# ictnlp/StreamSpeech

Hardware: AMD Instinct MI355X
Metric: real-time factor (RTFx = audio seconds / wall seconds) + utterances/sec, offline S2ST fr-en (higher is better)
Workload: dtype f32

## Files before the change

### include/streamspeech_hip.h

```cpp
#ifndef STREAMSPEECH_HIP_H
#define STREAMSPEECH_HIP_H

#include <stddef.h>
#include <stdint.h>

#ifdef __cplusplus
extern "C" {
#endif

#define SS_ABI_VERSION 2

typedef struct ss_model ss_model;
typedef struct ss_vocoder ss_vocoder;
typedef struct ss_scratch ss_scratch;
typedef struct ss_stream_pool ss_stream_pool;

typedef struct ss_config {
  int32_t input_feat, conv_channels, conv_kernel;
  int32_t enc_dim, enc_ffn, enc_heads, enc_layers, dw_kernel;
  int32_t src_vocab, tgt_vocab;
  int32_t mt_layers, dec_dim, dec_ffn, dec_heads;
  int32_t t2u_layers, unit_layers, unit_vocab, ctc_upsample;
  int32_t pad, eos, unk;
  int32_t max_rel_pos;
// ... 379 lines not shown
                          int64_t* h_attn_off, int64_t attn_capacity, int32_t* d_peak, float* d_stat);
int ss_batch_vocoder_tail(ss_vocoder* v, void* stream, int B, const int32_t* d_codes, const int32_t* h_K, const int32_t* h_n_new,
                          const int32_t* h_ctx, const int32_t* h_rf, int dur_prediction, float* d_out, int64_t out_capacity,
                          int32_t* h_win_first, int32_t* h_dur, int64_t* h_out_start, int64_t* h_n_out);
int ss_batch_vocoder_tail_spkr(ss_vocoder* v, void* stream, int B, const int32_t* d_codes, const int32_t* h_K, const int32_t* h_n_new,
                               const int32_t* h_ctx, const int32_t* h_rf, int dur_prediction, float* d_out, int64_t out_capacity,
                               int32_t* h_win_first, int32_t* h_dur, int64_t* h_out_start, int64_t* h_n_out,
                               const int32_t* h_spkr );

int ss_prof_enable(int cls_mask);
int ss_prof_enable_hi(int cls_mask);
int ss_prof_reset(void);
int ss_prof_read(int cls, double* h_ms_total, double* h_flops_total, int64_t* h_launches,
                 double* h_bytes_total);
int ss_prof_totals(int cls, double* h_flops_total, double* h_bytes_total, int64_t* h_launches);
int ss_prof_read_issued(int cls, double* h_issued_flops_total);
int ss_prof_shape_log(int on);
int ss_prof_shape_dump(char* buf, int cap);
int ss_prof_num_classes(void);
const char* ss_prof_class_name(int cls);

int ss_model_set_pack_invariant(ss_model* m, int on);
int ss_model_get_pack_invariant(ss_model* m);
int ss_debug_canon(int mode);

int ss_debug_last_logits(ss_model* m, void* stream, float* d_out, int64_t cap_floats, int* h_rows, int* h_cols);

int ss_op_ffn_fused(void* stream, const float* dX, int ldx, float* dY, int ldy, const float* ln_g, const float* ln_b,
                    const float* dW1, const float* db1, const float* dW2, const float* db2, float alpha,
                    const float* ln2_g, const float* ln2_b, int M, int D, int F);
int ss_debug_ffn(int grid, int row_tiles_per_wave, int enable);
int ss_debug_rtlin(int grid, int enable);
int ss_debug_conv_c64(int enable);
int ss_debug_conv_c32(int enable);
int ss_debug_conv_c16(int enable);
int64_t ss_debug_enc_step_launches(void);
int ss_op_ln_linear(void* stream, const float* dX, int ldx, const float* ln_g, const float* ln_b, const float* dW,
                    const float* dbias, const float* dR, int ldr, float* dC, int ldc, int M, int N, int K, int act, float alpha,
                    int glu);

int ss_debug_force_tile(int bm, int bn, int ks);
int ss_debug_sk_errors(void);
int ss_debug_attention_split(int v);
int ss_debug_attention_q16(int v);
int ss_debug_enc_step_inject_timeout(ss_model* m);
int ss_debug_scratch_audit(ss_scratch* sc, size_t* booked, size_t* held);
int ss_debug_mt_inject_timeout(ss_model* m);

int ss_op_conv_gemm(void* stream, const float* dA, int lda, const float* dW, const float* dbias,
                    const float* dR, int ldr, const float* dR2, int ldr2, float* dC, int ldc,
                    int M, int N, int Cin, int taps, int dil, int stride, int pad, int in_len,
                    int chunk, int in_act, float in_slope, int act, float alpha, float div, int glu);
typedef struct ss_op_conv_args {
  const float* A; const float* W; const float* bias; const float* R; const float* R2; float* C; float* C2;
  int32_t lda, ldc, ldr, ldr2, ldc2;
  int32_t M, N, Cin, taps, dil, stride, pad, in_len, chunk;
  int32_t in_act; float in_slope;
  int32_t act; float act_slope, alpha, div, c2_slope;
  int32_t glu;
  const int32_t* segs; int32_t nseg, max_seg_out;
  int32_t same_rows;
} ss_op_conv_args;
int ss_op_conv_gemm_ex(void* stream, const ss_op_conv_args* a);
int ss_op_conv_gemm_rows(void* stream, const ss_op_conv_args* a, int m_begin, const int32_t* seg_mb, const float* const* seg_A, int canon);
int ss_op_conv_pair(void* stream, const float* dA, int lda, const float* dW1, const float* db1, const float* dW2, const float* db2,
                    float* dC, int ldc, const float* dR2, int ldr2, float div, float* dC2, int ldc2, float c2_slope, int C, int taps,
// ... 121 lines not shown
```

### streamspeech_amd/csrc/conv_c64w.hip

```cpp
#include "slab_common.hpp"

#include <type_traits>

namespace ss {

using u32x4 = __attribute__((ext_vector_type(4))) unsigned;

#ifndef CW_TIMING
#define CW_TIMING 0
#endif
#if CW_TIMING
__device__ unsigned long long g_cw_dbg[1024 * 8];
#define CW_STAMP(k) do { if (t == 0) { const unsigned long long _n = __builtin_amdgcn_s_memtime(); cw_acc[k] += _n - cw_last; cw_last = _n; } } while (0)
#else
#define CW_STAMP(k) do { } while (0)
#endif

namespace {
constexpr int CW_MAXSEG = 256;
constexpr int CW_MAXROWS = 320;
[[maybe_unused]] constexpr int CW_NUM_RECORDS = 0x7ffffff0;
constexpr int cw_bme(int dil) { return dil == 1 ? 256 : dil == 3 ? 252 : 240; }
[[maybe_unused]] __host__ __device__ constexpr int cw_nc(int kind) { return kind == 0 ? 4 : kind == 1 ? 2 : 3; }
[[maybe_unused]] __host__ __device__ constexpr int cw_slot(int kind, int n) { return kind == 0 ? n : kind == 1 ? (n == 0 ? 0 : 3) : (n == 2 ? 3 : n); }
[[maybe_unused]] __host__ __device__ constexpr int cw_ja(int kind, int n) { return kind == 0 ? (n == 3 ? 1 : n) : kind == 1 ? n : (n == 0 ? 0 : 1); }
[[maybe_unused]] __host__ __device__ constexpr int cw_jb(int kind, int n) { return kind == 0 ? (n == 2 ? 1 : n == 3 ? 3 : 2) : kind == 1 ? n : (n == 2 ? 2 : 1); }
[[maybe_unused]] __host__ __device__ constexpr int cw_op(int kind, int n) { return kind == 0 ? (n == 1 ? 1 : -1) : kind == 1 ? 0 : (n == 1 ? 0 : -1); }
}

__global__ void wino_pack_kernel(const float* __restrict__ W, float* __restrict__ WW, int C, int taps, int groups) {
  const int n = C * groups * C;
  for (int idx = blockIdx.x * blockDim.x + threadIdx.x; idx < n; idx += gridDim.x * blockDim.x) {
    const int ci = idx % C, g = (idx / C) % groups, co = idx / (C * groups);
    const float* w = W + (size_t)co * taps * C + ci;
    const float w0 = 3 * g < taps ? w[(size_t)(3 * g) * C] : 0.f;
    const float w1 = 3 * g + 1 < taps ? w[(size_t)(3 * g + 1) * C] : 0.f;
    const float w2 = 3 * g + 2 < taps ? w[(size_t)(3 * g + 2) * C] : 0.f;
    float* o = WW + (size_t)co * groups * 4 * C + (size_t)g * 4 * C + ci;
    const int left = taps - 3 * g;
    if (left >= 3) {
      o[0] = w0;
      o[C] = 0.5f * ((w0 + w1) + w2);
      o[2 * C] = 0.5f * ((w0 - w1) + w2);
      o[3 * C] = w2;
    } else if (left == 2) {
      o[0] = w0; o[C] = w0 + w1; o[2 * C] = 0.f; o[3 * C] = w1;
    } else {
      o[0] = w0; o[C] = 0.f; o[2 * C] = 0.f; o[3 * C] = -w0;
    }
  }
}

template <int DIL, int CH, int TAIL>
__global__ __launch_bounds__(CH >= 128 ? 512 : 256, CH >= 128 ? 1 : CH == 64 ? 2 : 3) void conv_c64w_kernel(const GemmArgs p, const int groups, const int slab_rows) {
#if __HIP_DEVICE_COMPILE__
  constexpr int CS = CH == 256 ? 128 : CH;
  constexpr int KH = CH / CS;
  constexpr int C = CH, LDA = CS + 4, CT = CH >= 64 ? 4 : CH / 16, CB = CS / 16, RING = 2 * CT, TPR = CS / 4;
  constexpr int NT = CH >= 128 ? 512 : 256, RPP = NT / TPR;
  constexpr int NP = (CW_MAXROWS + RPP - 1) / RPP, NPC = CH == 256 ? 10 : NP < 20 ? NP : 20, BME = cw_bme(DIL), NPAIR = BME / 2;
  extern __shared__ __attribute__((aligned(16))) float smem[];
  float* sA = smem;
  int* s_blk = reinterpret_cast<int*>(smem + ((slab_rows * LDA + 3) & ~3));

  const int t = threadIdx.x, lane = t & 63;
  const int wave = __builtin_amdgcn_readfirstlane((t >> 6) & 3);
  const int cs = CH <= 64 ? 0 : __builtin_amdgcn_readfirstlane(t >> 8);
  const int colh = CH == 256 ? (int)((blockIdx.x >> 3) & 1) : 0;
  const int col0 = colh * 128 + cs * 64;
  const int r = lane & 15, g = lane >> 4;
  const int Kw = groups * 4 * C;

  SlabWalk<GemmArgs> w(p, s_blk, BME);
  __syncthreads();
  const int nblocks = w.nblocks();
  const float slope = p.in_act == ACT_LRELU ? p.in_slope : 1.0f;

  const __amdgpu_buffer_rsrc_t rsW = __builtin_amdgcn_make_buffer_rsrc((void*)p.W, 0, CW_NUM_RECORDS, 0x00020000);
  const int vo = (r * Kw + 4 * g) * 4;
  auto wload = [&](int idx, int cc, int ct, int kh) -> f32x4 {
    const int so = __builtin_amdgcn_readfirstlane(((col0 + ct * 16) * Kw + idx * C + kh * CS + cc * 16) * 4);
    const u32x4 v = __builtin_amdgcn_raw_buffer_load_b128(rsW, vo, so, 0);
    return f32x4{__uint_as_float(v[0]), __uint_as_float(v[1]), __uint_as_float(v[2]), __uint_as_float(v[3])};
  };

  int blk = CH == 256 ? (int)((blockIdx.x & 7) + 8 * (blockIdx.x >> 4)) : (int)blockIdx.x;
  const int blk_stride = CH == 256 ? (int)(gridDim.x >> 1) : (int)gridDim.x;
  if (blk >= nblocks) return;
  f32x4 ring[RING];
#pragma unroll
  for (int q = 0; q < RING; ++q) ring[q] = wload(q / CT, 0, q % CT, 0);

  int toff[2];
  bool pv[2];
#pragma unroll
  for (int i = 0; i < 2; ++i) {
    const int pp = wave * 32 + i * 16 + r;
    pv[i] = pp < NPAIR;
    const int pc = pv[i] ? pp : NPAIR - 1;
    toff[i] = 2 * DIL * (pc / DIL) + pc % DIL;
  }

#if CW_TIMING
  unsigned long long cw_acc[4] = {0, 0, 0, 0}, cw_last = __builtin_amdgcn_s_memtime(), cw_begin = cw_last, cw_blocks = 0;
#endif
  for (; blk < nblocks; blk += blk_stride) {
#if CW_TIMING
    ++cw_blocks;
#endif
    w.locate(blk, p.in_len);
    const int m0 = w.m0, seg_lo = w.seg_lo, seg_hi = w.seg_hi;
    const int m_hi = p.nseg > 0 ? seg_hi : min(seg_hi, p.M);
    const bool edge = (m0 - p.pad < seg_lo) || (m0 - p.pad + slab_rows > seg_hi);
    f32x4 acc[4][2][CT];
#pragma unroll
    for (int f = 0; f < 4; ++f)
#pragma unroll
      for (int i = 0; i < 2; ++i)
#pragma unroll
        for (int j = 0; j < CT; ++j) acc[f][i][j] = f32x4{0.f, 0.f, 0.f, 0.f};
#pragma unroll 1
    for (int kh = 0; kh < KH; ++kh) {
    const int kh_wrap = kh + 1 < KH ? kh + 1 : 0;
    __syncthreads();
    CW_STAMP(kh == 0 ? 3 : 1);
#pragma unroll 1
    for (int u0 = 0; u0 < NP; u0 += NPC) {
      f32x4 pre[NPC];
#pragma unroll
      for (int u = 0; u < NPC; ++u) {
        const int rho = t / TPR + RPP * (u0 + u);
        const int gc = min(max(m0 - p.pad + rho, seg_lo), seg_hi - 1);
        pre[u] = *reinterpret_cast<const f32x4*>(p.A + (size_t)gc * p.lda + kh * CS + (t % TPR) * 4);
      }
      float* dst = sA + (t / TPR + RPP * u0) * LDA + (t % TPR) * 4;
#pragma unroll
      for (int u = 0; u < NPC; ++u) {
        const int rho = t / TPR + RPP * (u0 + u);
        f32x4 v = pre[u];
        if (edge) {
          const int gin = m0 - p.pad + rho;
          const bool ok = gin >= seg_lo && gin < seg_hi;
#pragma unroll
          for (int e = 0; e < 4; ++e) v[e] = ok ? v[e] : 0.f;
        }
#pragma unroll
        for (int e = 0; e < 4; ++e) v[e] = fmaxf(v[e], v[e] * slope);
        if (rho < slab_rows) *reinterpret_cast<f32x4*>(dst + u * RPP * LDA) = v;
      }
    }
    __syncthreads();
    CW_STAMP(0);

    const float* pa0 = sA + toff[0] * LDA + 4 * g;
    const float* pa1 = sA + toff[1] * LDA + 4 * g;
    auto rd = [&](const float* base, int j, int cc) -> f32x4 { return *reinterpret_cast<const f32x4*>(base + j * DIL * LDA + cc * 16); };
    auto xform = [&](int op, const f32x4 a, const f32x4 b) -> f32x4 { return op == 1 ? a + b : op == 0 ? a : a - b; };
    f32x4 xa[2];
    xa[0] = xform(-1, rd(pa0, 0, 0), rd(pa0, 2, 0));
    xa[1] = xform(-1, rd(pa1, 0, 0), rd(pa1, 2, 0));
    auto group = [&](auto KIND, const int grp, const int kind_next, const float* pn0, const float* pn1, const int grp_next, const int kh_next) __attribute__((always_inline)) {
      constexpr int K = decltype(KIND)::value, NC = cw_nc(K), NS = CB * NC;
      static_assert(NS % 2 == 0 && NS >= 2, "ring slots keep their parity across groups");
#pragma unroll
      for (int ss = 0; ss < NS; ++ss) {
// ... 85 lines not shown
        for (int j = 0; j < CT; ++j) slab_epi_store<CH >= 128>(p, mrow[q], cole + j * 16, y[q * CT + j]);
      }
    }
    CW_STAMP(2);
  }
#if CW_TIMING
  if (t == 0) {
    unsigned long long* d = g_cw_dbg + (size_t)(blockIdx.x & 1023) * 8;
    d[0] = cw_acc[0]; d[1] = cw_acc[1]; d[2] = cw_acc[2]; d[3] = cw_acc[3]; d[4] = cw_blocks; d[5] = cw_begin; d[6] = __builtin_amdgcn_s_memtime(); d[7] = 1;
  }
#endif
#endif
}

#if CW_TIMING
extern "C" int ss_debug_cw_timing(unsigned long long* h_out, int cap_wgs) {
  const int n = cap_wgs < 1024 ? cap_wgs : 1024;
  if (hipMemcpyFromSymbol(h_out, HIP_SYMBOL(g_cw_dbg), (size_t)n * 8 * sizeof(unsigned long long)) != hipSuccess) return -1;
  static unsigned long long zeros[1024 * 8];
  (void)hipMemcpyToSymbol(HIP_SYMBOL(g_cw_dbg), zeros, sizeof(zeros));
  return n;
}
#endif

void conv_c64w_debug(int enable) { if (enable >= 0) dispatch_edit([enable](Dispatch& d) { d.c64w_on = enable ? 1 : 0; }); }
bool conv_c64w_enabled() { return disp().c64w_on != 0; }
void conv_c128w_debug(int enable) { if (enable >= 0) dispatch_edit([enable](Dispatch& d) { d.c128w_on = enable ? 1 : 0; }); }
bool conv_c128w_enabled() { return disp().c128w_on != 0; }

void conv_c256w_debug(int enable) { if (enable >= 0) dispatch_edit([enable](Dispatch& d) { d.c256w_on = enable ? 1 : 0; }); }
bool conv_c256w_enabled() { return disp().c256w_on != 0; }

static int cw_groups(const GemmArgs& a) { return (a.taps + 2) / 3; }
static size_t cw_lds(const GemmArgs& a, int ch) { return slab_lds_bytes(cw_bme(a.dil) + 3 * cw_groups(a) * a.dil, ch + 4, CW_MAXSEG); }

bool conv_c64w_eligible(const GemmArgs& a) {
  if (!disp().c64w_on || !a.Wwino || a.taps < disp().c64w_min_k || a.taps < 3 || (a.dil != 1 && a.dil != 3 && a.dil != 5) || a.C2) return false;
  if (a.pad != a.dil * (a.taps - 1) / 2) return false;
  if (a.taps <= 8 && a.taps > 3 && a.dil == 5) return false;
  const int slab_rows = cw_bme(a.dil) + 3 * cw_groups(a) * a.dil;
  return slab_rows <= CW_MAXROWS && 2 * cw_lds(a, 64) <= 158 * 1024 && (size_t)cw_groups(a) * 4 * 64 * 64 * 4 < 0x7ff00000ull;
}

bool conv_wide_winograd_eligible(const GemmArgs& a, int ch) {
  if (ch != 128 && ch != 256) return false;
  const Dispatch& d = disp();
  if (!(ch == 128 ? d.c128w_on : d.c256w_on) || !a.Wwino || !slab_conv_ok(a, ch)) return false;
  if (a.taps < 3 || (a.dil != 1 && a.dil != 3 && a.dil != 5) || a.pad != a.dil * (a.taps - 1) / 2) return false;
  if (a.nseg > CW_MAXSEG || a.M < (ch == 128 ? d.c128w_min_rows : d.c256w_min_rows) || !slab_rows_ok(a.M)) return false;
  if (ch == 256 && (size_t)256 * cw_groups(a) * 4 * 256 * 4 >= 0x7ff00000ull) return false;
  const int slab_rows = cw_bme(a.dil) + 3 * cw_groups(a) * a.dil;
  return slab_rows <= CW_MAXROWS && cw_lds(a, 128) <= 160 * 1024;
}

int launch_wino_pack(const float* W, float* WW, int C, int taps, hipStream_t stream) {
  const int groups = (taps + 2) / 3, n = C * groups * C;
  hipLaunchKernelGGL(wino_pack_kernel, dim3((n + 255) / 256), dim3(256), 0, stream, W, WW, C, taps, groups);
  SS_LAUNCH_CHECK();
  return SS_OK;
}

template <int DIL, int CH, int TAIL>
static int launch_cw_t(GemmArgs a, hipStream_t stream) {
  constexpr int BME = cw_bme(DIL);
  const int groups = cw_groups(a);
  const int slab_rows = BME + 3 * groups * DIL;
  const size_t lds = cw_lds(a, CH == 256 ? 128 : CH);
  SS_MAX_LDS_ONCE((&conv_c64w_kernel<DIL, CH, TAIL>), CH >= 128 ? 160 * 1024 : 96 * 1024);
  SkWorkspace* st = nullptr;
  int rc = sk_workspace_acquire(stream, &st);
  if (rc != SS_OK) return rc;
  int grid = slab_grid(CH >= 128 ? 1 : CH == 64 ? 2 : 3, st->cus, a.M, BME, a.nseg);
  if (CH == 256) {
    long long want = std::min<long long>(st->cus, 2 * ((slab_max_blocks(a.M, BME, a.nseg) + 7) / 8 * 8));
    if (disp().slab_grid_cap > 0) want = std::min<long long>(want, disp().slab_grid_cap);
    grid = (int)std::max<long long>(16, want / 16 * 16);
  }
  ProfRec rec{}; bool prof = false;
  rc = prof_begin(a, stream, CH == 64 ? PROF_CONV_C64W : CH == 128 ? PROF_CONV_C128W : CH == 256 ? PROF_CONV_C256W : PROF_CONV_C32W, rec, prof);
  if (rc != SS_OK) return rc;
  a.W = a.Wwino;
  hipLaunchKernelGGL((conv_c64w_kernel<DIL, CH, TAIL>), dim3(grid), dim3(CH >= 128 ? 512 : 256), lds, stream, a, groups, slab_rows);
  SS_LAUNCH_CHECK();
  return prof_end(stream, rec, prof);
}

template <int CH>
static int launch_cw(const GemmArgs& a, hipStream_t stream) {
  if (a.in_act != ACT_NONE && a.in_act != ACT_LRELU) return SS_ERR_ARG;
  const int key = a.dil * 10 + a.taps % 3;
  switch (key) {
    case 10: return launch_cw_t<1, CH, 0>(a, stream);
    case 11: return launch_cw_t<1, CH, 1>(a, stream);
    case 12: return launch_cw_t<1, CH, 2>(a, stream);
    case 30: return launch_cw_t<3, CH, 0>(a, stream);
    case 31: return launch_cw_t<3, CH, 1>(a, stream);
    case 32: return launch_cw_t<3, CH, 2>(a, stream);
    case 50: return launch_cw_t<5, CH, 0>(a, stream);
    case 51: return launch_cw_t<5, CH, 1>(a, stream);
    case 52: return launch_cw_t<5, CH, 2>(a, stream);
    default: return SS_ERR_ARG;
  }
}

int launch_conv_c64w(const GemmArgs& a, hipStream_t stream) {
  if (!conv_c64_eligible(a) || !conv_c64w_eligible(a)) return SS_ERR_ARG;
  return launch_cw<64>(a, stream);
}
void conv_c32w_debug(int enable) { if (enable >= 0) dispatch_edit([enable](Dispatch& d) { d.c32w_on = enable ? 1 : 0; }); }
bool conv_c32w_enabled() { return disp().c32w_on != 0; }
bool conv_c32w_eligible(const GemmArgs& a) {
  if (!disp().c32w_on || !a.Wwino || a.taps < 3 || (a.dil != 1 && a.dil != 3 && a.dil != 5) || a.C2) return false;
  if (a.pad != a.dil * (a.taps - 1) / 2) return false;
  const int slab_rows = cw_bme(a.dil) + 3 * cw_groups(a) * a.dil;
  return slab_rows <= CW_MAXROWS && 3 * cw_lds(a, 32) <= 158 * 1024;
// ... 16 lines not shown
```

### streamspeech_amd/csrc/debug_ops.hip

```cpp
#include "model_internal.hpp"

static int op_bind_wino(GemmArgs& a, void* stream) {
  static thread_local std::map<hipStream_t, DevBuf> wino_tmps;
  DevBuf& wino_tmp = wino_tmps[(hipStream_t)stream];
  const int N = a.N, Cin = a.Cin, taps = a.taps;
  if ((conv_c64w_enabled() && N == 64 && Cin == 64 && taps >= 3 && conv_c64_eligible(a)) ||
      (conv_c128w_enabled() && N == 128 && Cin == 128 && taps >= 3 && a.same_rows && !a.glu) ||
      (conv_c256w_enabled() && N == 256 && Cin == 256 && taps >= 3 && a.same_rows && !a.glu) ||
      (conv_c32w_enabled() && N == 32 && Cin == 32 && taps >= 3 && conv_c32_eligible(a))) {
    RET(wino_tmp.ensure((size_t)N * ((taps + 2) / 3) * 4 * N * sizeof(float)));
    RET(launch_wino_pack(a.W, wino_tmp.f(), N, taps, (hipStream_t)stream));
    a.Wwino = wino_tmp.f();
  }
  return SS_OK;
}

extern "C" int ss_op_conv_gemm(void* stream, const float* dA, int lda, const float* dW, const float* dbias,
                               const float* dR, int ldr, const float* dR2, int ldr2, float* dC, int ldc, int M,
                               int N, int Cin, int taps, int dil, int stride, int pad, int in_len, int chunk,
                               int in_act, float in_slope, int act, float alpha, float div, int glu) {
  GemmArgs a;
  a.A = dA; a.lda = lda; a.W = dW; a.bias = dbias; a.R = dR; a.ldr = ldr; a.R2 = dR2; a.ldr2 = ldr2; a.C = dC; a.ldc = ldc;
  a.M = M; a.N = N; a.Cin = Cin; a.taps = taps; a.dil = dil; a.stride = stride; a.pad = pad; a.in_len = in_len;
  a.chunk = chunk; a.in_act = in_act; a.in_slope = in_slope; a.act = act; a.alpha = alpha; a.div = div; a.glu = glu;
// ... 73 lines not shown
  if (!m->sc->dbg_logits || cap_floats < (int64_t)m->sc->dbg_rows * m->sc->dbg_cols) return SS_ERR_CAPACITY;
  SS_HIP_CHECK(hipMemcpyAsync(d_out, m->sc->dbg_logits, (size_t)m->sc->dbg_rows * m->sc->dbg_cols * sizeof(float), hipMemcpyDeviceToDevice,
                              (hipStream_t)stream));
  return SS_OK;
}

extern "C" int ss_op_ffn_fused(void* stream, const float* dX, int ldx, float* dY, int ldy, const float* ln_g, const float* ln_b,
                               const float* dW1, const float* db1, const float* dW2, const float* db2, float alpha,
                               const float* ln2_g, const float* ln2_b, int M, int D, int F) {
  return launch_ffn_fused(dX, ldx, dY, ldy, ln_g, ln_b, dW1, db1, dW2, db2, alpha, ln2_g, ln2_b, M, D, F, (hipStream_t)stream,
                          canon_mode() == CANON_SEQ);
}
extern "C" int ss_debug_canon(int mode) {
  if (mode < 0 || mode > 2) return SS_ERR_ARG;
  canon_debug_set(mode);
  return SS_OK;
}
extern "C" int ss_op_ln_linear(void* stream, const float* dX, int ldx, const float* ln_g, const float* ln_b, const float* dW,
                               const float* dbias, const float* dR, int ldr, float* dC, int ldc, int M, int N, int K, int act,
                               float alpha, int glu) {
  GemmArgs a;
  a.A = dX; a.lda = ldx; a.W = dW; a.bias = dbias; a.R = dR; a.ldr = ldr; a.C = dC; a.ldc = ldc;
  a.M = M; a.N = N; a.Cin = K; a.in_len = M; a.act = act; a.alpha = alpha; a.glu = glu; a.same_rows = 1;
  a.ln_g = ln_g; a.ln_b = ln_b;
  return launch_conv_gemm(a, (hipStream_t)stream);
}
extern "C" int ss_debug_conv_c64(int enable) {
  if (enable == 4 || enable == 5) { conv_c64w_debug(enable == 5); return SS_OK; }
  if (enable == 6 || enable == 7) { conv_c128w_debug(enable == 7); return SS_OK; }
  if (enable == 8 || enable == 9) { conv_c256w_debug(enable == 9); return SS_OK; }
  conv_c64_debug(enable);
  return SS_OK;
}
extern "C" int ss_debug_conv_c32(int enable) {
  if (enable == 4 || enable == 5) { conv_c32w_debug(enable == 5); return SS_OK; }
  conv_c32_debug(enable);
  return SS_OK;
}
extern "C" int ss_debug_conv_c16(int enable) { conv_c16_debug(enable); return SS_OK; }
extern "C" int64_t ss_debug_enc_step_launches(void) { return (int64_t)enc_step_launch_count(); }
extern "C" int ss_debug_scratch_audit(ss_scratch* sc, size_t* booked, size_t* held) {
  if (!sc || !booked || !held) return SS_ERR_ARG;
  size_t sum = 0;
  bool foreign = false;
  for (DevBuf* b : sc->all()) {
    sum += b->bytes;
    if (b->acct != &sc->acct) foreign = true;
  }
  *booked = sc->acct.used;
  *held = sum;
  return foreign ? SS_ERR_ARG : SS_OK;
}
extern "C" int ss_debug_rtlin(int grid, int enable) {
  if (grid < 0) return SS_ERR_ARG;
  rtlin_debug(grid, enable);
  return SS_OK;
}
extern "C" int ss_debug_ffn(int grid, int row_tiles_per_wave, int enable) {
  if (grid < 0 || row_tiles_per_wave < -1 || row_tiles_per_wave > 4) return SS_ERR_ARG;
  ffn_fused_debug_grid(grid);
  ffn_fused_debug_rows(row_tiles_per_wave);
  if (enable >= 0) dispatch_edit([enable](Dispatch& d) { d.ffn_fusion = enable ? 1 : 0; });
  return SS_OK;
}

extern "C" int ss_op_layernorm(void* stream, const float* dx, int ldx, float* dy, int ldy, const float* dg,
// ... 169 lines not shown
```

### streamspeech_amd/csrc/dispatch.hpp

```cpp
#pragma once
#include <functional>

namespace ss {

struct Dispatch {
  int attn_no_mfma = 0;
  int attn_q16 = 1;
  int attn_split = 0;
  int c16_off = 0, c32_off = 0, c64_off = 0;
  long long c16_min_rows = 131072, c32_min_rows = 65536, c64_min_rows = 32768;
  int c64w_on = 1, c128w_on = 1, c256w_on = 1, c32w_on = 1;
  int c64w_min_k = 3;
  long long c128w_min_rows = 65536, c256w_min_rows = 32768;
  int slab_grid_cap = 0;
  int sk_groups = 0;
  int ffn_force_g = 0;
  int ffn_wm = 3, ffn_wm_forced = 0;
  int ffn_fusion = 1;
  int ffn_min_rows = 1000;
  int force_bm = 0, force_bn = 0, force_ks = 0;
  double sk_min_flops = 4e9;
  int no_resblock_fusion = 0, no_pair_fusion = 0;
  int rt_off = 0, rt_min_rows = 193, rt_force_g = 0;
  long long rt_min_units = 4000;
  long long rt_kb_min_units = 256;
  int rt_kb_xmap = 1;
  int rt_kb_uw = 0;
};

const Dispatch& disp();
void dispatch_edit(const std::function<void(Dispatch&)>& fn);

struct CtxDispatch {
  Dispatch d;
  unsigned gen = 0xffffffffu;
  const Dispatch* refresh();
};
struct DispatchScope {
  explicit DispatchScope(const Dispatch* d);
  ~DispatchScope();
  const Dispatch* prev;
};

}
```

### streamspeech_amd/csrc/gemm.hip

```cpp
#include "gemm.hpp"

#include <atomic>
#include <cstdio>
#include <cstdlib>
#include <cstring>
#include <map>
#include <string>
#include <mutex>
#include <tuple>
#include <type_traits>
#include <utility>
#include <vector>

namespace ss {

using f32x4 = __attribute__((ext_vector_type(4))) float;

template <int BM, int BN, int BK, int WM, int WN, int KS, int PD, bool BLK = false>
__global__ __launch_bounds__(256 * KS) void conv_gemm_kernel(const GemmArgs p) {
  static_assert(WM * WN == 4, "4 waves per k-group");
  static_assert(!BLK || KS == 1, "the blocked chain is the KS = 1 form");
  constexpr int LDK = BK + 8;
  constexpr int WTM = BM / WM, WTN = BN / WN;
  constexpr int TM = WTM / 16, TN = WTN / 16;
// ... 761 lines not shown
  SkWorkspace* w = new SkWorkspace();
  std::lock_guard<std::mutex> lk(g_skw_mu);
  g_skw_live.push_back(w);
  return w;
}
void sk_workspace_free(SkWorkspace* w) {
  if (!w) return;
  {
    std::lock_guard<std::mutex> lk(g_skw_mu);
    for (size_t i = 0; i < g_skw_live.size(); ++i)
      if (g_skw_live[i] == w) { g_skw_live.erase(g_skw_live.begin() + i); break; }
  }
  if (w->ws) (void)hipFree(w->ws);
  if (w->sync1) (void)hipFree(w->sync1);
  if (w->sync2) (void)hipFree(w->sync2);
  if (w->sync3) (void)hipFree(w->sync3);
  if (w->dbg) (void)hipFree(w->dbg);
  delete w;
}
namespace {
std::mutex g_disp_mu;
std::atomic<unsigned> g_disp_gen{1};
Dispatch env_defaults() {
  Dispatch d;
  auto I = [](const char* k, int dflt) { const char* e = getenv(k); return e ? atoi(e) : dflt; };
  auto L = [](const char* k, long long dflt) { const char* e = getenv(k); return e ? atoll(e) : dflt; };
  d.attn_split = I("SS_ATTN_NO_SPLIT", 0) ? -1 : 0; d.attn_q16 = I("SS_ATTN_Q16", d.attn_q16);
  d.c16_off = I("SS_NO_CONV_C16", 0) ? 1 : 0; d.c32_off = I("SS_NO_CONV_C32", 0) ? 1 : 0; d.c64_off = I("SS_NO_CONV_C64", 0) ? 1 : 0;
  d.c16_min_rows = L("SS_CONV_C16_MIN_ROWS", d.c16_min_rows); d.c32_min_rows = L("SS_CONV_C32_MIN_ROWS", d.c32_min_rows);
  d.c64_min_rows = L("SS_CONV_C64_MIN_ROWS", d.c64_min_rows);
  d.c64w_on = I("SS_CONV_C64_WINOGRAD", 1); d.c128w_on = I("SS_CONV_C128_WINOGRAD", 1); d.c256w_on = I("SS_CONV_C256_WINOGRAD", 1);
  d.c32w_on = I("SS_CONV_C32_WINOGRAD", 1); d.c64w_min_k = I("SS_CONV_C64_WINOGRAD_MIN_K", 3);
  d.c128w_min_rows = L("SS_CONV_C128_MIN_ROWS", d.c128w_min_rows); d.c256w_min_rows = L("SS_CONV_C256_MIN_ROWS", d.c256w_min_rows);
  if (getenv("SS_FFN_WM")) { d.ffn_wm = I("SS_FFN_WM", 3); d.ffn_wm_forced = 1; }
  d.ffn_fusion = I("SS_NO_FFN_FUSION", 0) ? 0 : 1; d.ffn_min_rows = I("SS_FFN_MIN_ROWS", d.ffn_min_rows);
  if (getenv("SS_SK_MIN_GFLOP")) d.sk_min_flops = 1e9 * atof(getenv("SS_SK_MIN_GFLOP"));
  d.no_resblock_fusion = I("SS_NO_RESBLOCK_FUSION", 0); d.no_pair_fusion = I("SS_NO_PAIR_FUSION", 0);
  d.rt_off = I("SS_NO_RTLIN", 0) ? 1 : 0; d.rt_min_rows = I("SS_RTLIN_MIN_ROWS", d.rt_min_rows); d.rt_min_units = L("SS_RTLIN_MIN_UNITS", d.rt_min_units);
  d.rt_kb_min_units = L("SS_RTLIN_KB_MIN_UNITS", d.rt_kb_min_units); d.rt_kb_uw = I("SS_RTLIN_KB_UW", d.rt_kb_uw); d.rt_kb_xmap = I("SS_RTLIN_KB_XMAP", d.rt_kb_xmap);
  return d;
}
Dispatch& process_settings() { static Dispatch d = env_defaults(); return d; }
thread_local const Dispatch* t_disp = nullptr;
thread_local CtxDispatch t_disp_own;
}
void dispatch_edit(const std::function<void(Dispatch&)>& fn) {
  std::lock_guard<std::mutex> lk(g_disp_mu);
  fn(process_settings());
  g_disp_gen.fetch_add(1, std::memory_order_release);
}
void slab_debug(int grid, long long min_rows) {
  const Dispatch dflt = env_defaults();
  dispatch_edit([=](Dispatch& d) {
    d.slab_grid_cap = grid > 0 ? grid : 0;
    const bool set = min_rows >= 0;
    d.c16_min_rows = set ? min_rows : dflt.c16_min_rows; d.c32_min_rows = set ? min_rows : dflt.c32_min_rows;
    d.c64_min_rows = set ? min_rows : dflt.c64_min_rows;
    d.c128w_min_rows = set ? min_rows : dflt.c128w_min_rows; d.c256w_min_rows = set ? min_rows : dflt.c256w_min_rows;
  });
}
const Dispatch* CtxDispatch::refresh() {
  const unsigned now = g_disp_gen.load(std::memory_order_acquire);
  if (gen != now) {
    std::lock_guard<std::mutex> lk(g_disp_mu);
    d = process_settings();
    gen = g_disp_gen.load(std::memory_order_relaxed);
  }
  return &d;
}
const Dispatch& disp() { return t_disp ? *t_disp : *t_disp_own.refresh(); }
DispatchScope::DispatchScope(const Dispatch* d) : prev(t_disp) { t_disp = d; }
DispatchScope::~DispatchScope() { t_disp = prev; }

SkScope::SkScope(SkWorkspace* w) : prev(t_skw), prev_disp(t_disp) { t_skw = w; t_disp = w ? w->disp.refresh() : nullptr; }
SkScope::~SkScope() { t_skw = prev; t_disp = prev_disp; }

int sk_workspace_acquire(hipStream_t stream, SkWorkspace** out) {
  *out = nullptr;
  int dev = 0;
  SS_HIP_CHECK(hipGetDevice(&dev));
  SkWorkspace* w = t_skw;
  if (!w) {
    std::lock_guard<std::mutex> lk(g_skw_mu);
    SkWorkspace*& slot = g_skw_fallback[std::make_pair(dev, stream)];
    if (!slot) { slot = new SkWorkspace(); g_skw_live.push_back(slot); }
    w = slot;
  }
  if (!w->ws) {
    int cus = 0;
    SS_HIP_CHECK(hipDeviceGetAttribute(&cus, hipDeviceAttributeMultiprocessorCount, dev));
    if (cus <= 0) cus = 256;
    if (cus > 512) cus = 512;
// ... 198 lines not shown
```

### streamspeech_amd/csrc/gemm.hpp

```cpp
#pragma once
#include "common.hpp"
#include "dispatch.hpp"

namespace ss {

struct GemmArgs {
  const float* A = nullptr;
  const float* W = nullptr;
  const float* Wwino = nullptr;
  const void* Wf16 = nullptr;
  const float* bias = nullptr;
  const float* R = nullptr;
  const float* R2 = nullptr;
  float* C = nullptr;
  int lda = 0, ldc = 0, ldr = 0, ldr2 = 0;
  int M = 0, N = 0, Cin = 0;
  int taps = 1, dil = 1, stride = 1, pad = 0;
  int in_len = 0;
  int chunk = 0;
  int m_begin = 0;
  int in_act = ACT_NONE;
  float in_slope = 0.1f;
  int act = ACT_NONE;
  float alpha = 1.0f;
// ... 98 lines not shown
}
void slab_debug(int grid, long long min_rows);
bool slab_layout_ok(const GemmArgs& a);
bool slab_conv_ok(const GemmArgs& a, int c);
int device_cus(int& cus);

bool conv_slab_eligible(const GemmArgs& a);
int launch_conv_slab(const GemmArgs& a, hipStream_t stream);

bool conv_pair_eligible(int C, int taps, int dil, int lda, int ldc, int nseg, long long M);
int launch_conv_pair(const float* A, int lda, const float* W1, const float* b1, const float* W2, const float* b2, float* C,
                     int ldc, const float* R2, int ldr2, float div, float* C2, int ldc2, float c2_slope, int Cch, int taps,
                     int dil, int M, int in_len, float slope, const int* segs, int nseg, hipStream_t stream);

bool resblock_fused_eligible(int C, int taps, const int* dil, int ldx, int ldy, int nseg, long long M);
int launch_resblock_fused(const float* X, int ldx, const float* const* W1, const float* const* B1, const float* const* W2,
                          const float* const* B2, const int* dil, float* Y, int ldy, const float* R2, int ldr2, float div, int C,
                          int taps, int M, float slope, const int* segs, int nseg, hipStream_t stream);

bool conv_c64_eligible(const GemmArgs& a);
bool conv_c64_enabled();
int launch_conv_c64(const GemmArgs& a, hipStream_t stream);
bool conv_c64w_eligible(const GemmArgs& a);
int launch_conv_c64w(const GemmArgs& a, hipStream_t stream);
int launch_wino_pack(const float* W, float* WW, int C, int taps, hipStream_t stream);
void conv_c64w_debug(int enable);
bool conv_c64w_enabled();
bool conv_wide_winograd_eligible(const GemmArgs& a, int ch);
int launch_conv_c128w(const GemmArgs& a, hipStream_t stream);
void conv_c128w_debug(int enable);
bool conv_c128w_enabled();
int launch_conv_c256w(const GemmArgs& a, hipStream_t stream);
void conv_c256w_debug(int enable);
bool conv_c256w_enabled();
bool conv_c32w_eligible(const GemmArgs& a);
int launch_conv_c32w(const GemmArgs& a, hipStream_t stream);
void conv_c32w_debug(int enable);
bool conv_c32w_enabled();
void conv_c64_debug(int enable);

bool conv_c32_eligible(const GemmArgs& a);
bool conv_c32_enabled();
int launch_conv_c32(const GemmArgs& a, hipStream_t stream);
void conv_c32_debug(int enable);

bool conv_c16_eligible(const GemmArgs& a);
bool conv_c16_enabled();
int launch_conv_c16(const GemmArgs& a, hipStream_t stream);
void conv_c16_debug(int enable);

bool conv_f16_eligible(const GemmArgs& a);
bool conv_f16_geometry_ok(int C, int taps, int dil);
int launch_conv_f16(const GemmArgs& a, hipStream_t stream);
size_t f16_pack_halves(int C, int taps);
int launch_f16_pack(const float* W, void* Wf, int C, int taps, hipStream_t stream);

bool rtlin_eligible(const GemmArgs& a);
bool rtlin_shape_ok(const GemmArgs& a);
int launch_rtlin(const GemmArgs& a, hipStream_t stream);
void rtlin_debug(int grid, int enable);
bool rtlin_kb_shape_ok(const GemmArgs& a);
bool rtlin_kb_eligible(const GemmArgs& a);
int launch_rtlin_kb(const GemmArgs& a, hipStream_t stream);

bool ffn_fused_eligible(int D, int F, int act, int M, int ldx, int ldy, bool canon = false);
int launch_ffn_fused(const float* X, int ldx, float* Y, int ldy, const float* ln_g, const float* ln_b, const float* W1,
// ... 15 lines not shown
```

### streamspeech_amd/lib.py

```python
import ctypes as C
import os

_HERE = os.path.dirname(os.path.abspath(__file__))
LIB_PATH = os.environ.get("SS_HIP_LIB") or os.path.join(_HERE, "libstreamspeech_hip.so")


class SSConfig(C.Structure):
    _fields_ = [(n, C.c_int32) for n in (
        "input_feat", "conv_channels", "conv_kernel", "enc_dim", "enc_ffn", "enc_heads", "enc_layers",
        "dw_kernel", "src_vocab", "tgt_vocab", "mt_layers", "dec_dim", "dec_ffn", "dec_heads",
        "t2u_layers", "unit_layers", "unit_vocab", "ctc_upsample", "pad", "eos", "unk",
        "max_rel_pos", "max_tgt_pos")]


class SSVocoderConfig(C.Structure):
    _fields_ = [
        ("num_embeddings", C.c_int32), ("embedding_dim", C.c_int32), ("model_in_dim", C.c_int32),
        ("upsample_initial_channel", C.c_int32),
        ("n_up", C.c_int32), ("upsample_rates", C.c_int32 * 8), ("upsample_kernel_sizes", C.c_int32 * 8),
        ("n_res", C.c_int32), ("resblock_kernel_sizes", C.c_int32 * 4), ("resblock_dilations", (C.c_int32 * 3) * 4),
        ("dur_hidden", C.c_int32), ("dur_kernel", C.c_int32)]


_vp, _i, _f, _i64 = C.c_void_p, C.c_int, C.c_float, C.c_int64
# ... 219 lines not shown
                                                 C.POINTER(C.c_int32), _i64, C.POINTER(_i64), C.POINTER(SSMtSearchOpts)]),
    "ss_batch_fbank_frames": (_i, [_vp, _vp, _i, C.POINTER(_vp), C.POINTER(C.c_int32), C.POINTER(C.c_int32), _f,
                                   C.POINTER(_vp)]),
    "ss_batch_fbank_frames_sr": (_i, [_vp, _vp, _i, C.POINTER(_vp), C.POINTER(C.c_int32), C.POINTER(C.c_int32), C.POINTER(C.c_int32),
                                      C.POINTER(_vp), C.POINTER(C.c_int32), C.POINTER(C.c_int32), C.POINTER(C.c_int32), _f,
                                      C.POINTER(_vp)]),
    "ss_fbank_sr_rows": (_i, [_i64, _i, _i, _i, C.POINTER(C.c_int32), C.POINTER(C.c_int32)]),
    "ss_batch_t2u_units": (_i, [_vp, _vp, _i, _vp, _i, C.POINTER(C.c_int32), _i, _i, _vp, _vp, _vp]),
    "ss_batch_vocoder_forward": (_i, [_vp, _vp, _i, _vp, C.POINTER(C.c_int32), _i, _vp, _vp, _i64, _vp,
                                      C.POINTER(_i64), C.POINTER(_i64)]),
    "ss_batch_t2u_units_pad": (_i, [_vp, _vp, _i, _vp, _i, C.POINTER(C.c_int32), C.POINTER(C.c_int32), _i, _i, _vp, _vp, _vp]),
    "ss_batch_mt_features": (_i, [_vp, _vp, _i, _vp, C.POINTER(C.c_int32), C.POINTER(C.c_int32), C.POINTER(C.c_int32),
                                  C.POINTER(C.c_int32), _vp, _i]),
    "ss_batch_mt_attention": (_i, [_vp, _vp, _i, _vp, C.POINTER(C.c_int32), C.POINTER(C.c_int32), C.POINTER(C.c_int32),
                                   C.POINTER(C.c_int32), _vp, _i, _vp, C.POINTER(_i64), _i64, _vp, _vp]),
    "ss_batch_vocoder_tail": (_i, [_vp, _vp, _i, _vp, C.POINTER(C.c_int32), C.POINTER(C.c_int32), C.POINTER(C.c_int32),
                                   C.POINTER(C.c_int32), _i, _vp, _i64, C.POINTER(C.c_int32), C.POINTER(C.c_int32),
                                   C.POINTER(_i64), C.POINTER(_i64)]),
    "ss_prof_enable": (_i, [_i]),
    "ss_prof_enable_hi": (_i, [_i]),
    "ss_prof_reset": (_i, []),
    "ss_prof_read": (_i, [_i, C.POINTER(C.c_double), C.POINTER(C.c_double), C.POINTER(_i64), C.POINTER(C.c_double)]),
    "ss_prof_totals": (_i, [_i, C.POINTER(C.c_double), C.POINTER(C.c_double), C.POINTER(_i64)]),
    "ss_prof_read_issued": (_i, [_i, C.POINTER(C.c_double)]),
    "ss_prof_shape_log": (_i, [_i]),
    "ss_prof_shape_dump": (_i, [C.c_char_p, _i]),
    "ss_prof_num_classes": (_i, []),
    "ss_prof_class_name": (C.c_char_p, [_i]),
    "ss_debug_force_tile": (_i, [_i, _i, _i]),
    "ss_op_ffn_fused": (_i, [_vp, _vp, _i, _vp, _i, _vp, _vp, _vp, _vp, _vp, _vp, _f, _vp, _vp, _i, _i, _i]),
    "ss_debug_ffn": (_i, [_i, _i, _i]),
    "ss_debug_rtlin": (_i, [_i, _i]),
    "ss_debug_conv_c64": (_i, [_i]),
    "ss_debug_conv_c32": (_i, [_i]),
    "ss_debug_conv_c16": (_i, [_i]),
    "ss_debug_enc_step_launches": (_i64, []),
    "ss_debug_scratch_audit": (_i, [_vp, C.POINTER(C.c_size_t), C.POINTER(C.c_size_t)]),
    "ss_op_ln_linear": (_i, [_vp, _vp, _i, _vp, _vp, _vp, _vp, _vp, _i, _vp, _i, _i, _i, _i, _i, _f, _i]),
    "ss_debug_last_logits": (_i, [_vp, _vp, _vp, _i64, C.POINTER(_i), C.POINTER(_i)]),
    "ss_debug_sk_errors": (_i, []),
    "ss_debug_attention_split": (_i, [_i]),
    "ss_debug_attention_q16": (_i, [_i]),
    "ss_op_conv_gemm": (_i, [_vp, _vp, _i, _vp, _vp, _vp, _i, _vp, _i, _vp, _i, _i, _i, _i, _i, _i, _i, _i, _i, _i,
                             _i, _f, _i, _f, _f, _i]),
    "ss_op_conv_gemm_ex": (_i, [_vp, C.POINTER(SSOpConvArgs)]),
    "ss_op_conv_gemm_rows": (_i, [_vp, C.POINTER(SSOpConvArgs), _i, _vp, _vp, _i]),
    "ss_op_conv_pair": (_i, [_vp, _vp, _i, _vp, _vp, _vp, _vp, _vp, _i, _vp, _i, _f, _vp, _i, _f, _i, _i, _i, _i, _i, _f, _vp, _i]),
    "ss_op_resblock_fused": (_i, [_vp, _vp, _i, _vp, _vp, _vp, _vp, _vp, _vp, _i, _vp, _i, _f, _i, _i, _i, _f, _vp, _i]),
    "ss_debug_slab": (_i, [_i, C.c_longlong]),
    "ss_op_conv_f16": (_i, [_vp, _vp, _vp, _vp, _vp, _vp, _vp, _vp, _i, _i, _i, _i, _i, _f, _i, _f, _vp, _i]),
    "ss_op_layernorm": (_i, [_vp, _vp, _i, _vp, _i, _vp, _vp, _i, _i, _f]),
    "ss_op_attention": (_i, [_vp, _vp, _i, _vp, _i, _vp, _i, _vp, _i, _i, _i, _i, _f, _i, _i, _vp, _i, _vp, _vp]),
    "ss_op_attention_ex": (_i, [_vp, C.POINTER(SSOpAttnArgs)]),
    "ss_op_attention_probs": (_i, [_vp, C.POINTER(SSOpAttnProbsArgs)]),
    "ss_op_attention_pool": (_i, [_vp, C.POINTER(SSOpPoolAttnArgs)]),
    "ss_debug_attention_no_mfma": (_i, [_i]),
    "ss_op_dwconv_bn_silu": (_i, [_vp, _vp, _i, _vp, _i, _vp, _i, _vp, _vp, _vp, _vp, _f, _i, _i, _i]),
    "ss_op_dwconv_bn_silu_ex": (_i, [_vp, _vp, _i, _vp, _i, _vp, _i, _vp, _vp, _vp, _vp, _f, _i, _i, _i, _vp, _i, _i]),
    "ss_op_pool_dwconv": (_i, [_vp, _vp, _vp, _i, _vp, _vp, _i, _vp, _vp, _vp, _vp, _f, _i, _vp, _i, _i]),
    "ss_op_pool_gather_rows": (_i, [_vp, _vp, _vp, _vp, _i, _i, _vp, _vp, _i, _i]),
    "ss_op_pool_gather_ids": (_i, [_vp, _vp, _vp, _vp, _i, _vp, _vp, _i, _i]),
    "ss_op_pool_stack_rows": (_i, [_vp, _vp, _vp, _i, _vp, _vp, _i, _i]),
    "ss_op_masked_argmax": (_i, [_vp, _vp, _i, _i, _i, _i, _i, _i, _i, _vp, _vp, _i, _i, _vp, _i]),
    "ss_op_ctc_collapse": (_i, [_vp, _vp, _i, _i, _i, _vp, _vp, _vp, _vp, _i]),
    "ss_op_masked_argmax_lprob": (_i, [_vp, _vp, _i, _i, _i, _i, _i, _i, _vp, _vp]),
    "ss_op_ctc_collapse_spans": (_i, [_vp, _vp, _vp, _i, _i, _i, _vp, _vp, _vp, _vp, _vp, _vp, _i]),
# ... 64 lines not shown
```

Measured before the change: 6403.

## Add half-height 128-row slab variant for 256-channel Winograd conv kernel

```diff
diff --git a/include/streamspeech_hip.h b/include/streamspeech_hip.h
--- a/include/streamspeech_hip.h
+++ b/include/streamspeech_hip.h
@@ -435,6 +435,7 @@
 int ss_debug_ffn(int grid, int row_tiles_per_wave, int enable);
 int ss_debug_rtlin(int grid, int enable);
 int ss_debug_conv_c64(int enable);
+int ss_debug_conv_c256_rows(int rows);
 int ss_debug_conv_c32(int enable);
 int ss_debug_conv_c16(int enable);
 int64_t ss_debug_enc_step_launches(void);
diff --git a/streamspeech_amd/csrc/conv_c64w.hip b/streamspeech_amd/csrc/conv_c64w.hip
--- a/streamspeech_amd/csrc/conv_c64w.hip
+++ b/streamspeech_amd/csrc/conv_c64w.hip
@@ -19,8 +19,9 @@
 namespace {
 constexpr int CW_MAXSEG = 256;
 constexpr int CW_MAXROWS = 320;
+constexpr int CW_MAXROWS_128 = 192;
 [[maybe_unused]] constexpr int CW_NUM_RECORDS = 0x7ffffff0;
-constexpr int cw_bme(int dil) { return dil == 1 ? 256 : dil == 3 ? 252 : 240; }
+constexpr int cw_bme(int dil, int rows = 256) { return rows == 128 ? (dil == 1 ? 128 : dil == 3 ? 126 : 120) : (dil == 1 ? 256 : dil == 3 ? 252 : 240); }
 [[maybe_unused]] __host__ __device__ constexpr int cw_nc(int kind) { return kind == 0 ? 4 : kind == 1 ? 2 : 3; }
 [[maybe_unused]] __host__ __device__ constexpr int cw_slot(int kind, int n) { return kind == 0 ? n : kind == 1 ? (n == 0 ? 0 : 3) : (n == 2 ? 3 : n); }
 [[maybe_unused]] __host__ __device__ constexpr int cw_ja(int kind, int n) { return kind == 0 ? (n == 3 ? 1 : n) : kind == 1 ? n : (n == 0 ? 0 : 1); }
@@ -51,22 +52,24 @@
   }
 }
 
-template <int DIL, int CH, int TAIL>
+template <int DIL, int CH, int TAIL, int ROWS = 256>
 __global__ __launch_bounds__(CH >= 128 ? 512 : 256, CH >= 128 ? 1 : CH == 64 ? 2 : 3) void conv_c64w_kernel(const GemmArgs p, const int groups, const int slab_rows) {
 #if __HIP_DEVICE_COMPILE__
   constexpr int CS = CH == 256 ? 128 : CH;
   constexpr int KH = CH / CS;
   constexpr int C = CH, LDA = CS + 4, CT = CH >= 64 ? 4 : CH / 16, CB = CS / 16, RING = 2 * CT, TPR = CS / 4;
   constexpr int NT = CH >= 128 ? 512 : 256, RPP = NT / TPR;
-  constexpr int NP = (CW_MAXROWS + RPP - 1) / RPP, NPC = CH == 256 ? 10 : NP < 20 ? NP : 20, BME = cw_bme(DIL), NPAIR = BME / 2;
+  static_assert(ROWS == 256 || (ROWS == 128 && CH == 256), "half-height blocks: the 256-channel form only");
+  constexpr int NP = ((ROWS == 128 ? CW_MAXROWS_128 : CW_MAXROWS) + RPP - 1) / RPP, NPC = CH == 256 ? 10 : NP < 20 ? NP : 20;
+  constexpr int BME = cw_bme(DIL, ROWS), NPAIR = BME / 2;
   extern __shared__ __attribute__((aligned(16))) float smem[];
   float* sA = smem;
   int* s_blk = reinterpret_cast<int*>(smem + ((slab_rows * LDA + 3) & ~3));
 
   const int t = threadIdx.x, lane = t & 63;
-  const int wave = __builtin_amdgcn_readfirstlane((t >> 6) & 3);
-  const int cs = CH <= 64 ? 0 : __builtin_amdgcn_readfirstlane(t >> 8);
-  const int colh = CH == 256 ? (int)((blockIdx.x >> 3) & 1) : 0;
+  const int wave = __builtin_amdgcn_readfirstlane((t >> 6) & (ROWS == 128 ? 1 : 3));
+  const int cs = CH <= 64 ? 0 : __builtin_amdgcn_readfirstlane(ROWS == 128 ? t >> 7 : t >> 8);
+  const int colh = CH == 256 && ROWS == 256 ? (int)((blockIdx.x >> 3) & 1) : 0;
   const int col0 = colh * 128 + cs * 64;
   const int r = lane & 15, g = lane >> 4;
   const int Kw = groups * 4 * C;
@@ -84,8 +87,9 @@
     return f32x4{__uint_as_float(v[0]), __uint_as_float(v[1]), __uint_as_float(v[2]), __uint_as_float(v[3])};
   };
 
-  int blk = CH == 256 ? (int)((blockIdx.x & 7) + 8 * (blockIdx.x >> 4)) : (int)blockIdx.x;
-  const int blk_stride = CH == 256 ? (int)(gridDim.x >> 1) : (int)gridDim.x;
+  constexpr bool HALVES = CH == 256 && ROWS == 256;
+  int blk = HALVES ? (int)((blockIdx.x & 7) + 8 * (blockIdx.x >> 4)) : (int)blockIdx.x;
+  const int blk_stride = HALVES ? (int)(gridDim.x >> 1) : (int)gridDim.x;
   if (blk >= nblocks) return;
   f32x4 ring[RING];
 #pragma unroll
@@ -112,6 +116,7 @@
     const int m0 = w.m0, seg_lo = w.seg_lo, seg_hi = w.seg_hi;
     const int m_hi = p.nseg > 0 ? seg_hi : min(seg_hi, p.M);
     const bool edge = (m0 - p.pad < seg_lo) || (m0 - p.pad + slab_rows > seg_hi);
+    const int row_hi = ROWS == 128 ? min(seg_hi, m0 - p.pad + slab_rows) : seg_hi;
     f32x4 acc[4][2][CT];
 #pragma unroll
     for (int f = 0; f < 4; ++f)
@@ -125,12 +130,12 @@
     __syncthreads();
     CW_STAMP(kh == 0 ? 3 : 1);
 #pragma unroll 1
-    for (int u0 = 0; u0 < NP; u0 += NPC) {
+    for (int u0 = 0; u0 < NP && (ROWS != 128 || u0 * RPP < slab_rows); u0 += NPC) {
       f32x4 pre[NPC];
 #pragma unroll
       for (int u = 0; u < NPC; ++u) {
         const int rho = t / TPR + RPP * (u0 + u);
-        const int gc = min(max(m0 - p.pad + rho, seg_lo), seg_hi - 1);
+        const int gc = min(max(m0 - p.pad + rho, seg_lo), row_hi - 1);
         pre[u] = *reinterpret_cast<const f32x4*>(p.A + (size_t)gc * p.lda + kh * CS + (t % TPR) * 4);
       }
       float* dst = sA + (t / TPR + RPP * u0) * LDA + (t % TPR) * 4;
@@ -282,7 +287,10 @@
 bool conv_c256w_enabled() { return disp().c256w_on != 0; }
 
 static int cw_groups(const GemmArgs& a) { return (a.taps + 2) / 3; }
-static size_t cw_lds(const GemmArgs& a, int ch) { return slab_lds_bytes(cw_bme(a.dil) + 3 * cw_groups(a) * a.dil, ch + 4, CW_MAXSEG); }
+static size_t cw_lds(const GemmArgs& a, int ch, int rows = 256) { return slab_lds_bytes(cw_bme(a.dil, rows) + 3 * cw_groups(a) * a.dil, ch + 4, CW_MAXSEG); }
+static bool cw_rows128(const GemmArgs& a) {
+  return disp().c256w_rows == 128 && cw_bme(a.dil, 128) + 3 * cw_groups(a) * a.dil <= CW_MAXROWS_128;
+}
 
 bool conv_c64w_eligible(const GemmArgs& a) {
   if (!disp().c64w_on || !a.Wwino || a.taps < disp().c64w_min_k || a.taps < 3 || (a.dil != 1 && a.dil != 3 && a.dil != 5) || a.C2) return false;
@@ -299,6 +307,7 @@
   if (a.taps < 3 || (a.dil != 1 && a.dil != 3 && a.dil != 5) || a.pad != a.dil * (a.taps - 1) / 2) return false;
   if (a.nseg > CW_MAXSEG || a.M < (ch == 128 ? d.c128w_min_rows : d.c256w_min_rows) || !slab_rows_ok(a.M)) return false;
   if (ch == 256 && (size_t)256 * cw_groups(a) * 4 * 256 * 4 >= 0x7ff00000ull) return false;
+  if (ch == 256 && cw_rows128(a)) return cw_lds(a, 128, 128) <= 160 * 1024;
   const int slab_rows = cw_bme(a.dil) + 3 * cw_groups(a) * a.dil;
   return slab_rows <= CW_MAXROWS && cw_lds(a, 128) <= 160 * 1024;
 }
@@ -310,18 +319,21 @@
   return SS_OK;
 }
 
-template <int DIL, int CH, int TAIL>
+template <int DIL, int CH, int TAIL, int ROWS = 256>
 static int launch_cw_t(GemmArgs a, hipStream_t stream) {
-  constexpr int BME = cw_bme(DIL);
+  if constexpr (CH == 256 && ROWS == 256) {
+    if (cw_rows128(a)) return launch_cw_t<DIL, CH, TAIL, 128>(a, stream);
+  }
+  constexpr int BME = cw_bme(DIL, ROWS);
   const int groups = cw_groups(a);
   const int slab_rows = BME + 3 * groups * DIL;
-  const size_t lds = cw_lds(a, CH == 256 ? 128 : CH);
-  SS_MAX_LDS_ONCE((&conv_c64w_kernel<DIL, CH, TAIL>), CH >= 128 ? 160 * 1024 : 96 * 1024);
+  const size_t lds = cw_lds(a, CH == 256 ? 128 : CH, ROWS);
+  SS_MAX_LDS_ONCE((&conv_c64w_kernel<DIL, CH, TAIL, ROWS>), CH >= 128 ? 160 * 1024 : 96 * 1024);
   SkWorkspace* st = nullptr;
   int rc = sk_workspace_acquire(stream, &st);
   if (rc != SS_OK) return rc;
   int grid = slab_grid(CH >= 128 ? 1 : CH == 64 ? 2 : 3, st->cus, a.M, BME, a.nseg);
-  if (CH == 256) {
+  if (CH == 256 && ROWS == 256) {
     long long want = std::min<long long>(st->cus, 2 * ((slab_max_blocks(a.M, BME, a.nseg) + 7) / 8 * 8));
     if (disp().slab_grid_cap > 0) want = std::min<long long>(want, disp().slab_grid_cap);
     grid = (int)std::max<long long>(16, want / 16 * 16);
@@ -330,7 +342,7 @@
   rc = prof_begin(a, stream, CH == 64 ? PROF_CONV_C64W : CH == 128 ? PROF_CONV_C128W : CH == 256 ? PROF_CONV_C256W : PROF_CONV_C32W, rec, prof);
   if (rc != SS_OK) return rc;
   a.W = a.Wwino;
-  hipLaunchKernelGGL((conv_c64w_kernel<DIL, CH, TAIL>), dim3(grid), dim3(CH >= 128 ? 512 : 256), lds, stream, a, groups, slab_rows);
+  hipLaunchKernelGGL((conv_c64w_kernel<DIL, CH, TAIL, ROWS>), dim3(grid), dim3(CH >= 128 ? 512 : 256), lds, stream, a, groups, slab_rows);
   SS_LAUNCH_CHECK();
   return prof_end(stream, rec, prof);
 }
diff --git a/streamspeech_amd/csrc/debug_ops.hip b/streamspeech_amd/csrc/debug_ops.hip
--- a/streamspeech_amd/csrc/debug_ops.hip
+++ b/streamspeech_amd/csrc/debug_ops.hip
@@ -129,6 +129,7 @@
   conv_c64_debug(enable);
   return SS_OK;
 }
+extern "C" int ss_debug_conv_c256_rows(int rows) { return conv_c256w_rows_debug(rows); }
 extern "C" int ss_debug_conv_c32(int enable) {
   if (enable == 4 || enable == 5) { conv_c32w_debug(enable == 5); return SS_OK; }
   conv_c32_debug(enable);
diff --git a/streamspeech_amd/csrc/dispatch.hpp b/streamspeech_amd/csrc/dispatch.hpp
--- a/streamspeech_amd/csrc/dispatch.hpp
+++ b/streamspeech_amd/csrc/dispatch.hpp
@@ -12,6 +12,7 @@
   int c64w_on = 1, c128w_on = 1, c256w_on = 1, c32w_on = 1;
   int c64w_min_k = 3;
   long long c128w_min_rows = 65536, c256w_min_rows = 32768;
+  int c256w_rows = 128;
   int slab_grid_cap = 0;
   int sk_groups = 0;
   int ffn_force_g = 0;
diff --git a/streamspeech_amd/csrc/gemm.hip b/streamspeech_amd/csrc/gemm.hip
--- a/streamspeech_amd/csrc/gemm.hip
+++ b/streamspeech_amd/csrc/gemm.hip
@@ -817,6 +817,7 @@
   d.c64w_on = I("SS_CONV_C64_WINOGRAD", 1); d.c128w_on = I("SS_CONV_C128_WINOGRAD", 1); d.c256w_on = I("SS_CONV_C256_WINOGRAD", 1);
   d.c32w_on = I("SS_CONV_C32_WINOGRAD", 1); d.c64w_min_k = I("SS_CONV_C64_WINOGRAD_MIN_K", 3);
   d.c128w_min_rows = L("SS_CONV_C128_MIN_ROWS", d.c128w_min_rows); d.c256w_min_rows = L("SS_CONV_C256_MIN_ROWS", d.c256w_min_rows);
+  if (const int r = I("SS_CONV_C256_ROWS", d.c256w_rows); r == 128 || r == 256) d.c256w_rows = r;
   if (getenv("SS_FFN_WM")) { d.ffn_wm = I("SS_FFN_WM", 3); d.ffn_wm_forced = 1; }
   d.ffn_fusion = I("SS_NO_FFN_FUSION", 0) ? 0 : 1; d.ffn_min_rows = I("SS_FFN_MIN_ROWS", d.ffn_min_rows);
   if (getenv("SS_SK_MIN_GFLOP")) d.sk_min_flops = 1e9 * atof(getenv("SS_SK_MIN_GFLOP"));
@@ -843,6 +844,12 @@
     d.c64_min_rows = set ? min_rows : dflt.c64_min_rows;
     d.c128w_min_rows = set ? min_rows : dflt.c128w_min_rows; d.c256w_min_rows = set ? min_rows : dflt.c256w_min_rows;
   });
+}
+int conv_c256w_rows_debug(int rows) {
+  if (rows != 0 && rows != 128 && rows != 256) return SS_ERR_ARG;
+  const int dflt = env_defaults().c256w_rows;
+  dispatch_edit([=](Dispatch& d) { d.c256w_rows = rows ? rows : dflt; });
+  return SS_OK;
 }
 const Dispatch* CtxDispatch::refresh() {
   const unsigned now = g_disp_gen.load(std::memory_order_acquire);
diff --git a/streamspeech_amd/csrc/gemm.hpp b/streamspeech_amd/csrc/gemm.hpp
--- a/streamspeech_amd/csrc/gemm.hpp
+++ b/streamspeech_amd/csrc/gemm.hpp
@@ -154,6 +154,7 @@
 bool conv_c128w_enabled();
 int launch_conv_c256w(const GemmArgs& a, hipStream_t stream);
 void conv_c256w_debug(int enable);
+int conv_c256w_rows_debug(int rows);
 bool conv_c256w_enabled();
 bool conv_c32w_eligible(const GemmArgs& a);
 int launch_conv_c32w(const GemmArgs& a, hipStream_t stream);
diff --git a/streamspeech_amd/lib.py b/streamspeech_amd/lib.py
--- a/streamspeech_amd/lib.py
+++ b/streamspeech_amd/lib.py
@@ -275,6 +275,7 @@
     "ss_debug_ffn": (_i, [_i, _i, _i]),
     "ss_debug_rtlin": (_i, [_i, _i]),
     "ss_debug_conv_c64": (_i, [_i]),
+    "ss_debug_conv_c256_rows": (_i, [_i]),
     "ss_debug_conv_c32": (_i, [_i]),
     "ss_debug_conv_c16": (_i, [_i]),
     "ss_debug_enc_step_launches": (_i64, []),
```

Result: faster. 6469 (median of 6 runs) (+1.0%).
